# volivan239/raytracing-course-hw

Measured on AMD Instinct MI355X. Metric: Msamples/sec at 1920x1080x256spp, higher is better.
Workload: dtype f32; 1 GPU; synth_room_v1_1920x1080x256; scene=synth_room_v1 (seed 20241223), triangles=268816, emissive_triangles=4204, width=1920, height=1080, spp=256, ray_depth=6, parallelism=pixel tiles 32x32 round-robin over 1 GPU(s), bvh_nodes=265605, bvh_depth=24, light_bvh_depth=19, device_bytes=120573816

## Files before the change

raytracing-course-hw_amd/csrc/host/device_build.h:

```cpp
#pragma once
#include "../device/rt_types.h"
#include <cstdint>
#include <hip/hip_runtime.h>

namespace rtamd {

struct DeviceTree {
    GpuNode *nodes = nullptr;
    uint32_t *order = nullptr;
    uint8_t *last = nullptr;
    uint32_t n_nodes = 0, depth = 0;
    float build_ms = 0.f;
};

DeviceTree build_tree_on_device(const float *d_boxes, uint32_t n, float abs_pad, uint32_t max_depth);
void free_device_tree(DeviceTree &t);

void gather_records(const void *d_in, void *d_out, const DeviceTree &t, uint32_t n, uint32_t elem_bytes, int mark_word_offset, bool or_into_word = false);

void join_root_box(const GpuNode *d_nodes, float lo[3], float hi[3]);

GpuNode4Q *widen_nodes(const GpuNode *d_nodes, uint32_t n, const NodeGrid &grid, uint32_t &n_out, uint32_t &depth_out);

}
```

raytracing-course-hw_amd/csrc/rtamd_build.hip:

```cpp
#include "device/rt_bvh_build.h"
#include "device/rt_node_grid.h"
#include "host/device_build.h"
#include "host/fold_nodes.h"
#include "host/hip_check.h"
#include <cmath>
#include <stdexcept>
#include <string>
#include <vector>

namespace rtamd {

namespace {
__global__ void gather16_kernel(const float4 *in, float4 *out, const uint32_t *order, const uint8_t *last, uint32_t n, uint32_t quads, int mark_word, bool or_mark) {
    const uint32_t i = blockIdx.x * blockDim.x + threadIdx.x;
    if (i >= n) return;
    const float4 *src = in + (size_t)order[i] * quads;
    float4 *dst = out + (size_t)i * quads;
    for (uint32_t q = 0; q < quads; q++) dst[q] = src[q];
    if (mark_word >= 0) {
        uint32_t *w = reinterpret_cast<uint32_t *>(dst) + mark_word;
        const uint32_t mark = last[i] ? 1u : 0u;
        *w = or_mark ? ((*w & ~1u) | mark) : mark;
    }
}
}

void join_root_box(const GpuNode *d_nodes, float lo[3], float hi[3]) {
    GpuNode root;
    HIP_CHECK(hipMemcpy(&root, d_nodes, sizeof root, hipMemcpyDeviceToHost));
    auto join = [&](const float *l, const float *h) { for (int k = 0; k < 3; k++) { if (l[k] < lo[k]) lo[k] = l[k]; if (h[k] > hi[k]) hi[k] = h[k]; } };
    if ((uint32_t)root.child0 != 0xFFFFFFFFu) join(root.lo0, root.hi0);
    if ((uint32_t)root.child1 != 0xFFFFFFFFu) join(root.lo1, root.hi1);
}

GpuNode4Q *widen_nodes(const GpuNode *d_nodes, uint32_t n, const NodeGrid &grid, uint32_t &n_out, uint32_t &depth_out) {
    std::vector<GpuNode> nodes(n ? n : 1);
    if (n) HIP_CHECK(hipMemcpy(nodes.data(), d_nodes, (size_t)n * sizeof(GpuNode), hipMemcpyDeviceToHost));
    else { GpuNode e{}; e.child0 = e.child1 = (int32_t)0xFFFFFFFFu; nodes[0] = e; }
    std::vector<GpuNode4Q> wide;
    fold_nodes(nodes, grid, wide, depth_out);
    n_out = (uint32_t)wide.size();
    GpuNode4Q *out = nullptr;
    HIP_CHECK(hipMalloc((void **)&out, wide.size() * sizeof(GpuNode4Q)));
    if (hipMemcpy(out, wide.data(), wide.size() * sizeof(GpuNode4Q), hipMemcpyHostToDevice) != hipSuccess) { (void)hipFree(out); throw std::runtime_error("widen_nodes: upload failed"); }
    return out;
}

DeviceTree build_tree_on_device(const float *d_boxes, uint32_t n, float abs_pad, uint32_t max_depth) {
    DeviceTree t;
    if (n == 0) throw std::runtime_error("build_tree_on_device: no primitives");
    dev::BvbView B{};
    if (max_depth < 8 || max_depth > BVB_MAX_DEPTH) throw std::runtime_error("build_tree_on_device: max_depth out of range");
    B.boxes = d_boxes; B.n = n; B.abs_pad = abs_pad; B.max_depth = max_depth;
    const size_t max_open = (size_t)n / 2 + 2, max_nodes = 2 * (size_t)n + 2;
    std::vector<void *> temps;
    auto alloc = [&](size_t bytes, bool temp) { void *p = nullptr; HIP_CHECK(hipMalloc(&p, bytes)); if (temp) temps.push_back(p); return p; };
    try {
        B.prim_node = (uint32_t *)alloc((size_t)n * 4, true);
        B.nodes = (dev::BvbNode *)alloc(max_nodes * sizeof(dev::BvbNode), true);
        B.bins = (uint32_t *)alloc(max_open * BVB_NODE_BIN_WORDS * 4, true);
        B.dec = (dev::BvbDecision *)alloc(max_open * sizeof(dev::BvbDecision), true);
        B.open_cur = (uint32_t *)alloc(max_open * 4, true);
        B.open_next = (uint32_t *)alloc(max_open * 4, true);
        B.st = (dev::BvbState *)alloc(sizeof(dev::BvbState), true);
        t.order = B.order = (uint32_t *)alloc((size_t)n * 4, false);
        t.last = (uint8_t *)alloc((size_t)n, false);
        hipEvent_t e0, e1;
        HIP_CHECK(hipEventCreate(&e0)); HIP_CHECK(hipEventCreate(&e1));
        hipStream_t stream = 0;
        HIP_CHECK(hipEventRecord(e0, stream));
        HIP_CHECK(hipMemsetAsync(B.nodes, 0, 2 * sizeof(dev::BvbNode), stream));
        HIP_CHECK(hipMemsetAsync(B.bins, 0, max_open * BVB_NODE_BIN_WORDS * 4, stream));
        HIP_CHECK(hipMemsetAsync(t.last, 0, n, stream));
        const uint32_t prim_blocks = (n + 255) / 256, prim_wgs = (n + BVB_THREADS - 1) / BVB_THREADS, open_blocks = (uint32_t)((max_open + 255) / 256);
        hipLaunchKernelGGL(dev::bvb_init_kernel, dim3(prim_blocks), dim3(256), 0, stream, B);
        hipLaunchKernelGGL(dev::bvb_root_kernel, dim3(1), dim3(64), 0, stream, B);
        for (int level = 0; level <= (int)max_depth; level++) {
            hipLaunchKernelGGL(dev::bvb_bin_kernel, dim3(prim_wgs), dim3(BVB_THREADS), 0, stream, B);
            hipLaunchKernelGGL(dev::bvb_split_kernel, dim3(open_blocks), dim3(256), 0, stream, B);
            hipLaunchKernelGGL(dev::bvb_number_kernel, dim3(1), dim3(BVB_THREADS), 0, stream, B);
            hipLaunchKernelGGL(dev::bvb_assign_kernel, dim3(prim_wgs), dim3(BVB_THREADS), 0, stream, B);
            std::swap(B.open_cur, B.open_next);
            hipLaunchKernelGGL(dev::bvb_next_level_kernel, dim3(1), dim3(64), 0, stream, B);
            if ((level & 7) == 7) {
                dev::BvbState st;
                HIP_CHECK(hipMemcpyAsync(&st, B.st, sizeof st, hipMemcpyDeviceToHost, stream));
                HIP_CHECK(hipStreamSynchronize(stream));
                if (st.n_open == 0) break;
            }
        }
        hipLaunchKernelGGL(dev::bvb_layout_kernel, dim3(1), dim3(BVB_THREADS), 0, stream, B);
        dev::BvbState st;
        HIP_CHECK(hipMemcpyAsync(&st, B.st, sizeof st, hipMemcpyDeviceToHost, stream));
        HIP_CHECK(hipStreamSynchronize(stream));
        if (st.n_open != 0 || st.n_leaf_slots != n || st.n_nodes > max_nodes)
            throw std::runtime_error("build_tree_on_device: inconsistent tree (open " + std::to_string(st.n_open) + ", slots " + std::to_string(st.n_leaf_slots) + " of " + std::to_string(n) + ")");
        t.n_nodes = st.n_inner ? st.n_inner : 1u;
        t.depth = st.max_depth;
        t.nodes = B.out_nodes = (GpuNode *)alloc((size_t)t.n_nodes * sizeof(GpuNode), false);
        const uint32_t node_blocks = (st.n_nodes + 255) / 256;
        hipLaunchKernelGGL(dev::bvb_place_kernel, dim3(prim_blocks), dim3(256), 0, stream, B);
        hipLaunchKernelGGL(dev::bvb_emit_kernel, dim3(node_blocks), dim3(256), 0, stream, B);
        hipLaunchKernelGGL(dev::bvb_marks_kernel, dim3(node_blocks), dim3(256), 0, stream, B, t.last);
        HIP_CHECK(hipEventRecord(e1, stream));
        HIP_CHECK(hipStreamSynchronize(stream));
        HIP_CHECK(hipGetLastError());
        HIP_CHECK(hipEventElapsedTime(&t.build_ms, e0, e1));
        (void)hipEventDestroy(e0); (void)hipEventDestroy(e1);
    } catch (...) {
        for (void *p : temps) (void)hipFree(p);
        free_device_tree(t);
        throw;
    }
    for (void *p : temps) (void)hipFree(p);
    return t;
}

void free_device_tree(DeviceTree &t) {
    if (t.nodes) (void)hipFree(t.nodes);
    if (t.order) (void)hipFree(t.order);
    if (t.last) (void)hipFree(t.last);
    t.nodes = nullptr; t.order = nullptr; t.last = nullptr;
}

void gather_records(const void *d_in, void *d_out, const DeviceTree &t, uint32_t n, uint32_t elem_bytes, int mark_word_offset, bool or_into_word) {
    if (elem_bytes % 16) throw std::runtime_error("gather_records: record size must be a multiple of 16");
    hipLaunchKernelGGL(gather16_kernel, dim3((n + 255) / 256), dim3(256), 0, 0, (const float4 *)d_in, (float4 *)d_out, t.order, t.last, n, elem_bytes / 16, mark_word_offset, or_into_word);
    HIP_CHECK(hipGetLastError());
}

}
```

raytracing-course-hw_amd/csrc/rtamd_scene.hip:

```cpp
#include <hip/hip_runtime.h>
#include <cmath>
#include <cstdio>
#include <cstdlib>
#include <cstring>
#include <memory>
#include <string>
#include <vector>
#include "../../include/rtamd.h"
#include "host/host_scene.h"
#include "host/png.h"
#include "host/scene_prep.h"
#include "host/shared_prep.h"
#include "host/device_build.h"
#include "host/knobs.h"
#include "host/rt_scene.h"
#include "device/rt_node_grid.h"

namespace rtamd {
static thread_local std::string g_last_error;
void set_error(const std::string &msg) { g_last_error = msg; }
}
using namespace rtamd;

namespace {

struct OwnedTree {
    DeviceTree t;
    ~OwnedTree() { free_device_tree(t); }
};

template <class Rec>
DeviceTree build_leaf_ordered(rt_scene *s, const float *d_boxes, const Rec *d_records, uint32_t n, float box_pad, uint32_t depth_cap,
                              int mark_word, bool or_into_word, const Rec *&gathered) {
    OwnedTree tree;
    tree.t = build_tree_on_device(d_boxes, n, box_pad, depth_cap);
    OwnedDev out;
    HIP_CHECK(hipMalloc(&out.p, (size_t)n * sizeof(Rec)));
    gather_records(d_records, out.p, tree.t, n, sizeof(Rec), mark_word, or_into_word);
    HIP_CHECK(hipDeviceSynchronize());
    s->allocations.reserve(s->allocations.size() + 2);
    s->allocations.push_back(tree.t.nodes);
    s->allocations.push_back(out.p);
    gathered = (const Rec *)out.release();
    DeviceTree t = tree.t;
    t.order = nullptr; t.last = nullptr;
    tree.t.nodes = nullptr;
    return t;
}

void make_walk_nodes(rt_scene *s, const float cam_pos[3], const GpuNode *nodes, uint32_t n_nodes, const GpuNode *light_nodes, uint32_t n_light_nodes,
                     bool join_light_root, NodeGrid &grid, const GpuNode4Q *&nodes4, const GpuNode4Q *&light_nodes4, uint64_t &bytes) {
    float glo[3], ghi[3];
    for (int k = 0; k < 3; k++) glo[k] = ghi[k] = cam_pos[k];
    join_root_box(nodes, glo, ghi);
    if (join_light_root) join_root_box(light_nodes, glo, ghi);
    grid = make_node_grid(glo, ghi);
    uint32_t n4 = 0, n4l = 0, depth4 = 0;
    s->allocations.push_back(widen_nodes(nodes, n_nodes, grid, n4, depth4));
    nodes4 = (const GpuNode4Q *)s->allocations.back();
    s->allocations.push_back(widen_nodes(light_nodes, n_light_nodes, grid, n4l, depth4));
    light_nodes4 = (const GpuNode4Q *)s->allocations.back();
    bytes += ((uint64_t)n4 + n4l) * sizeof(GpuNode4Q);
}

template <class View> void set_camera(View &V, const rt_scene_desc &desc) {
    for (int k = 0; k < 3; k++) {
        V.cam_pos[k] = desc.camera.position[k]; V.cam_right[k] = desc.camera.right[k];
        V.cam_up[k] = desc.camera.up[k]; V.cam_fwd[k] = desc.camera.forward[k];
        V.bg[k] = desc.bg_color[k];
    }
}

int finish_scene(std::unique_ptr<rt_scene> &s, rt_scene **out, uint64_t bytes, double t0, double t1) {
    HIP_CHECK(hipMalloc((void **)&s->d_work_counter, 64));
    s->allocations.push_back(s->d_work_counter);
    HIP_CHECK(hipMalloc((void **)&s->d_counters, CNT_BYTES));
    s->allocations.push_back(s->d_counters);
    HIP_CHECK(hipEventCreate(&s->ev_start));
    HIP_CHECK(hipEventCreate(&s->ev_stop));
    HIP_CHECK(hipDeviceSynchronize());
    s->info.device_bytes = bytes;
    s->info.prep_ms = t1 - t0; s->info.upload_ms = now_ms() - t1;
    *out = s.release();
    return RT_OK;
}

struct Uploader {
    rt_scene *s;
    uint64_t bytes = 0;
    template <class T> const T *operator()(const std::vector<T> &v) { s->allocations.push_back((void *)upload(v, bytes)); return (const T *)s->allocations.back(); }
};
template <class View> void upload_ref_trees(View &V, const PreparedTrees &P, Uploader &up) { V.ref_nodes = up(P.ref_nodes); V.ref_light_nodes = up(P.ref_light_nodes); }
void report_trees(rt_scene *s, const rt_scene_desc *desc, const PreparedTrees &P, uint32_t n_lights, uint32_t n_nodes, uint32_t bvh_depth) {
    s->light_order = P.light_order;
    s->info.n_triangles = desc->n_triangles; s->info.n_lights = n_lights;
    s->info.n_bvh_nodes = n_nodes; s->info.n_light_bvh_nodes = (uint32_t)P.light_nodes.size();
    s->info.bvh_depth = bvh_depth; s->info.light_bvh_depth = P.light_bvh_depth;
}

template <class View> void set_triangle_view(View &V, const rt_scene_desc &desc, const PreparedTriangles &P, uint32_t components) {
    V.box_c2 = P.box_c2; V.box_c2x = 1.25f * P.box_c2;
    V.cull_k = (float)env_float("RTAMD_CULL_K", 0.0078125);
    V.n_tris = desc.n_triangles;
    V.n_lights = (uint32_t)P.light_order.size();
    V.n_components = components + (V.n_lights ? 1u : 0u);
    V.n_lights_f = (float)V.n_lights; V.n_components_f = (float)V.n_components;
    set_camera(V, desc);
    V.tan_fov_y = (float)std::tan((double)(desc.camera.fov_y / 2));
}

int create_txt(const rt_scene_desc *desc, std::unique_ptr<rt_scene> &s, rt_scene **out, double t0) {
    PreparedSceneTxt T;
    prepare_scene_txt(*desc, T);
    PreparedScene5 P5;
    prepare_scene_hw5(*desc, P5);
    Uploader up{s.get()};
    s->txt_has_triangles = T.has_triangles;
    SceneViewTxt &V = s->viewt;
    V.prims = up(T.prims);
    V.n_prims = desc->n_primitives;
    set_camera(V, *desc);
    V.tan_fov_x = (float)std::tan((double)(desc->camera.fov_x / 2));
    V.tan_fov_x_f = tanf(desc->camera.fov_x / 2);
    V.n_lights = desc->n_lights;
    if (desc->n_lights) V.lights = up(T.lights);
    for (int k = 0; k < 3; k++) V.ambient[k] = desc->ambient_light[k];
    V.n_light_prims = (uint32_t)T.light_prims.size();
    if (!T.light_prims.empty()) V.light_prims = up(T.light_prims);
    SceneView5 &V5 = s->view5;
    V5.nodes = up(P5.nodes);
    V5.figs = up(P5.figs);
    V5.light_nodes = up(P5.light_nodes);
    upload_ref_trees(V5, P5, up);
    if (!P5.lights.empty()) V5.lights = up(P5.lights);
    V5.n_figs = (uint32_t)P5.figs.size(); V5.n_nonplanes = P5.n_nonplanes; V5.n_lights = (uint32_t)P5.lights.size();
    set_camera(V5, *desc);
    V5.tan_fov_x = V.tan_fov_x;
    report_trees(s.get(), desc, P5, V5.n_lights, (uint32_t)P5.nodes.size(), P5.bvh_depth);
    s->flavor = RT_INTEGRATOR_HW3;
    return finish_scene(s, out, up.bytes, t0, t0);
}

int create_hw6(const rt_scene_desc *desc, std::unique_ptr<rt_scene> &s, rt_scene **out, double t0) {
    const bool tree_on_device = desc->n_triangles >= 64 && !env_flag("RTAMD_HOST_BVH");
    PreparedScene6 P6;
    prepare_scene_hw6(*desc, P6, tree_on_device);
    uint32_t bvh_depth = P6.bvh_depth, n_nodes = (uint32_t)P6.nodes.size();
    double t1 = now_ms();
    Uploader up{s.get()};
    SceneView6 &V = s->view6;
    if (tree_on_device) {
        uint64_t scratch = 0;
        OwnedDev d_load(upload(P6.tris, up.bytes));
        OwnedDev d_boxes(upload(P6.boxes8, scratch));
        const DeviceTree t = build_leaf_ordered(s.get(), (const float *)d_boxes.p, (const Tri6 *)d_load.p, desc->n_triangles, P6.box_pad, 28,
                                                13, false, V.tris);
        V.nodes = t.nodes;
        up.bytes += (uint64_t)t.n_nodes * sizeof(GpuNode);
        bvh_depth = t.depth;
        n_nodes = t.n_nodes;
        s->info.bvh_build_ms = t.build_ms; s->info.bvh_on_device = 1;
    } else {
        V.nodes = up(P6.nodes);
        V.tris = up(P6.tris);
    }
    if (bvh_depth > RT6_STACK_SIZE - 2 || P6.light_bvh_depth > RT6_STACK_SIZE - 2 || P6.fast_light_bvh_depth > RT6_STACK_SIZE - 2)
        return fail(RT_ERR_LIMIT, "scene BVH deeper than the kernel's traversal stack (" + std::to_string(bvh_depth) + "/" +
                                      std::to_string(P6.light_bvh_depth) + ")");
    s->hw6_lds_stack = bvh_depth <= RT6_LDS_STACK && P6.fast_light_bvh_depth <= RT6_LDS_STACK;
    s->hw6_pt_stack = bvh_depth <= P6_STACK && P6.fast_light_bvh_depth <= P6_STACK;
    V.light_nodes = up(P6.light_nodes);
    V.lights = up(P6.lights);
    V.fast_light_nodes = up(P6.fast_light_nodes);
    V.fast_lights = up(P6.fast_lights);
    V.light_ref = up(P6.light_ref);
    upload_ref_trees(V, P6, up);
    V.ref_tris = up(P6.ref_tris);
    V.tri_box = up(P6.tri_box);
    set_triangle_view(V, *desc, P6, 1u);
    V.exact_boxes = env_flag("RTAMD_NO_EXACT_BOXES") ? 0u : 1u;
    V.light_sep = up(P6.light_sep);
    V.materials = up(P6.materials);
    s->view.tan_fov_y = V.tan_fov_y;
    s->flavor = RT_INTEGRATOR_HW6;
    make_walk_nodes(s.get(), V.cam_pos, V.nodes, n_nodes, V.fast_light_nodes, (uint32_t)P6.fast_light_nodes.size(), true,
                    V.grid, V.nodes4, V.fast_light_nodes4, up.bytes);
    report_trees(s.get(), desc, P6, V.n_lights, n_nodes, bvh_depth);
    return finish_scene(s, out, up.bytes, t0, t1);
}

int create_hw8(const rt_scene_desc *desc, std::unique_ptr<rt_scene> &s, rt_scene **out, double t0, SharedPrep *shared) {
    if (desc->build_flags & ~RT_BUILD_DEVICE_BVH) return fail(RT_ERR_INVALID_ARG, "rt_scene_create: unknown build_flags");
    const bool fast_build = (desc->build_flags & RT_BUILD_DEVICE_BVH) && desc->n_triangles >= 64;
    const bool walk_tree_on_device = desc->n_triangles >= 64 && (fast_build || !env_flag("RTAMD_HOST_BVH"));
    PreparedScene P_local;
    if (shared) std::call_once(shared->once, [&] { try { prepare_scene(*desc, shared->P, fast_build); } catch (...) { shared->error = std::current_exception(); } });
    else prepare_scene(*desc, P_local, fast_build);
    if (shared && shared->error) std::rethrow_exception(shared->error);
    const PreparedScene &P = shared ? shared->P : P_local;
    uint32_t bvh_depth = P.bvh_depth, n_nodes = (uint32_t)P.nodes.size();
    double t1 = now_ms();
    Uploader up{s.get()};
    SceneView &V = s->view;
    V.tri_isect = up(P.isect);
    V.tri_shade = up(P.shade);
    V.tri_box = up(P.tri_box);
    if (walk_tree_on_device) {
        const uint32_t n = desc->n_triangles;
        uint64_t scratch = 0;
        OwnedDev d_walk_box;
        if (!P.walk_box.empty()) d_walk_box.p = upload(P.walk_box, scratch);
        const DeviceTree t = build_leaf_ordered(s.get(), d_walk_box.p ? (const float *)d_walk_box.p : V.tri_box, V.tri_isect, n, P.box_pad, P8_STACK,
                                                11, true, V.tri_walk);
        V.nodes = t.nodes;
        up.bytes += (uint64_t)t.n_nodes * sizeof(GpuNode) + (uint64_t)n * sizeof(TriIsect);
        bvh_depth = t.depth;
        n_nodes = t.n_nodes;
        s->info.bvh_build_ms = t.build_ms; s->info.bvh_on_device = 1;
    } else {
        V.nodes = up(P.nodes);
        V.tri_walk = V.tri_isect;
    }
    if (P.bvh_depth > RT_STACK_SIZE - 2)
        return fail(RT_ERR_LIMIT, "the reference's scene BVH is deeper than the exact walk's stack (" + std::to_string(P.bvh_depth) + ")");
    if (bvh_depth > RT_STACK_SIZE - 2 || P.light_bvh_depth > RT_STACK_SIZE - 2)
        return fail(RT_ERR_LIMIT, "scene BVH deeper than the kernel's traversal stack (" + std::to_string(bvh_depth) + "/" +
                                      std::to_string(P.light_bvh_depth) + ")");
    V.light_nodes = up(P.light_nodes);
    V.light_sep = up(P.light_sep);
    upload_ref_trees(V, P, up);
    set_triangle_view(V, *desc, P, 2u);
    V.box_c2x *= (float)env_float("RTAMD_C2X_SCALE", 1.0);
    V.exact_boxes = (env_flag("RTAMD_NO_EXACT_BOXES") || fast_build) ? 0u : 1u;
    if (env_flag("RTAMD_DIAG_LOOKBEHIND_ONLY")) V.exact_boxes = 2u;
    V.n_tripwire_groups = (V.exact_boxes != 1u || env_flag("RTAMD_NO_TRIPWIRES")) ? 0u : P.n_tripwire_groups;
    V.tripwires = V.n_tripwire_groups ? up(P.tripwires) : nullptr;
    V.lights = up(P.lights);
    uint32_t n_light_walk_nodes = 0;
    {
        const uint32_t nl = (uint32_t)P.lights.size();
        const LightRec *ordered = nullptr;
        std::vector<LightRec> tagged = P.lights;
        for (uint32_t i = 0; i < nl; i++) tagged[i].isect.pad = (i << 1) | (tagged[i].isect.pad ? 1u : 0u);
        if (nl >= 64 && !env_flag("RTAMD_HOST_LIGHT_BVH")) {
            uint64_t scratch = 0;
            OwnedDev d_tagged(upload(tagged, up.bytes));
            OwnedDev d_lbox(upload(P.light_walk_box, scratch));
            const DeviceTree lt = build_leaf_ordered(s.get(), (const float *)d_lbox.p, (const LightRec *)d_tagged.p, nl, P.box_pad, 16,
                                                     11, true, ordered);
            V.light_walk_nodes = lt.nodes;
            up.bytes += (uint64_t)lt.n_nodes * sizeof(GpuNode);
            s->light_walk_depth = lt.depth;
            n_light_walk_nodes = lt.n_nodes;
        } else {
            V.light_walk_nodes = V.light_nodes;
            n_light_walk_nodes = (uint32_t)P.light_nodes.size();
            ordered = up(tagged);
            s->light_walk_depth = P.light_bvh_depth;
        }
        OwnedDev whole(s->allocations.back());
        s->allocations.pop_back();
        const size_t n_rec = nl ? nl : 1u;
        char *pair = nullptr;
        HIP_CHECK(hipMalloc((void **)&pair, n_rec * sizeof(LightRec)));
        s->allocations.push_back(pair);
        char *rest = pair + n_rec * sizeof(TriIsect);
        HIP_CHECK(hipMemcpy2D(pair, sizeof(TriIsect), ordered, sizeof(LightRec), sizeof(TriIsect), n_rec, hipMemcpyDeviceToDevice));
        HIP_CHECK(hipMemcpy2D(rest, sizeof(LightRest), (const char *)ordered + sizeof(TriIsect), sizeof(LightRec), sizeof(LightRest), n_rec, hipMemcpyDeviceToDevice));
        V.lights_walk_test = (const TriIsect *)pair;
        V.lights_walk_rest = (const LightRest *)rest;
    }
    V.materials = up(P.materials);
    V.images = up(P.images);
    V.texels = up(P.texels);
    V.srgb_lut = up(std::vector<float>(P.srgb_lut, P.srgb_lut + 256));
    V.n_nodes = n_nodes;
    V.last_level_emission_only = 1;
    for (uint32_t i = 0; i < desc->n_materials; i++) {
        const rt_material &m = desc->materials[i];
        if (!(m.metallic_factor >= 0 && m.metallic_factor <= 1 && m.base_color[0] >= 0 && m.base_color[1] >= 0 && m.base_color[2] >= 0))
            V.last_level_emission_only = 0;
    }
    if (env_flag("RTAMD_NO_LAST_LEVEL_SHORTCUT")) V.last_level_emission_only = 0;
    V.env_image = P.env_image;
    if (!walk_arrays_fit(desc->n_triangles, V.n_lights, n_nodes, n_light_walk_nodes))
        return fail(RT_ERR_LIMIT, "the scene's triangles, lights or tree nodes do not fit the walkers' 32-bit offsets (2^24 records, 4 GiB per array)");
    make_walk_nodes(s.get(), V.cam_pos, V.nodes, n_nodes, V.light_walk_nodes, n_light_walk_nodes, n_light_walk_nodes != 0,
                    V.grid, V.nodes4, V.light_walk_nodes4, up.bytes);
    report_trees(s.get(), desc, P, V.n_lights, n_nodes, bvh_depth);
    return finish_scene(s, out, up.bytes, t0, t1);
}

}

int rtamd::scene_create_shared(const rt_scene_desc *desc, rt_scene **out, rtamd::SharedPrep *shared) {
    if (!desc || !out) return fail(RT_ERR_INVALID_ARG, "rt_scene_create: null argument");
    if (desc->struct_size != sizeof(rt_scene_desc)) return fail(RT_ERR_INVALID_ARG, "rt_scene_create: struct_size mismatch (ABI skew)");
    *out = nullptr;
    int ndev = 0;
    if (hipGetDeviceCount(&ndev) != hipSuccess || ndev == 0)
        return fail(RT_ERR_NO_DEVICE, "rt_scene_create: no HIP device available (this library has no CPU fallback)");
    return guarded("", [&]() -> int {
        std::unique_ptr<rt_scene> s(new rt_scene());
        HIP_CHECK(hipGetDevice(&s->device));
        hipDeviceProp_t prop;
        HIP_CHECK(hipGetDeviceProperties(&prop, s->device));
        s->n_cus = prop.multiProcessorCount > 0 ? prop.multiProcessorCount : 256;
        const double t0 = now_ms();
        if (desc->n_triangles == 0 && (desc->n_primitives > 0 || (desc->camera.fov_x != 0.f && desc->camera.fov_y == 0.f))) return create_txt(desc, s, out, t0);
        if (desc->n_triangles && !desc->normals) return create_hw6(desc, s, out, t0);
        return create_hw8(desc, s, out, t0, shared);
    });
}

extern "C" {

const char *rt_last_error(void) { return g_last_error.c_str(); }

int rt_scene_create(const rt_scene_desc *desc, rt_scene **out) { return rtamd::scene_create_shared(desc, out, nullptr); }

void rt_scene_destroy(rt_scene *scene) { delete scene; }

int rt_scene_get_info(const rt_scene *scene, rt_scene_info *info) {
    if (!scene || !info) return fail(RT_ERR_INVALID_ARG, "rt_scene_get_info: null argument");
    *info = scene->info;
    return RT_OK;
}

int rt_scene_get_light_order(const rt_scene *scene, uint32_t *out, uint32_t capacity) {
    if (!scene || (!out && capacity)) return fail(RT_ERR_INVALID_ARG, "rt_scene_get_light_order: null argument");
    if (capacity < scene->light_order.size()) return fail(RT_ERR_INVALID_ARG, "rt_scene_get_light_order: buffer too small");
    memcpy(out, scene->light_order.data(), scene->light_order.size() * sizeof(uint32_t));
    return (int)scene->light_order.size();
}

int rt_host_prepare_orders(const rt_scene_desc *desc, int integrator, uint32_t *figure_order, uint32_t figure_capacity,
                           uint32_t *light_order, uint32_t light_capacity) {
    if (!desc || desc->struct_size != sizeof(rt_scene_desc)) return fail(RT_ERR_INVALID_ARG, "rt_host_prepare_orders: bad desc");
    return guarded("rt_host_prepare_orders: ", [&]() -> int {
        auto answer = [&](const PreparedTrees &P) -> int {
            if ((figure_order && figure_capacity < P.figure_order.size()) || (light_order && light_capacity < P.light_order.size())) return fail(RT_ERR_INVALID_ARG, "rt_host_prepare_orders: buffer too small");
            if (figure_order) memcpy(figure_order, P.figure_order.data(), P.figure_order.size() * sizeof(uint32_t));
            if (light_order) memcpy(light_order, P.light_order.data(), P.light_order.size() * sizeof(uint32_t));
            return (int)P.light_order.size();
        };
        if (integrator == RT_INTEGRATOR_HW8 || integrator == RT_INTEGRATOR_HW7) { PreparedScene P; prepare_scene(*desc, P); return answer(P); }
        if (integrator == RT_INTEGRATOR_HW6) { PreparedScene6 P; prepare_scene_hw6(*desc, P); return answer(P); }
        if (integrator == RT_INTEGRATOR_HW5) { PreparedScene5 P; prepare_scene_hw5(*desc, P); return answer(P); }
        return fail(RT_ERR_UNSUPPORTED, "rt_host_prepare_orders: integrator must be HW5, HW6, HW7 or HW8");
    });
}

int rt_unshard(const rt_render_params *p, const void *shard_buf, size_t elem_size, void *full_image) {
    if (!p || !shard_buf || !full_image || (elem_size != 1 && elem_size != 4)) return fail(RT_ERR_INVALID_ARG, "rt_unshard: bad argument");
    return guarded("rt_unshard: ", [&]() -> int {
    RenderView R{};
    std::string err;
    if (!resolve_tiles(p, R, err)) return fail(RT_ERR_INVALID_ARG, "rt_unshard: " + err);
    const uint8_t *src = (const uint8_t *)shard_buf;
    uint8_t *dst = (uint8_t *)full_image;
    size_t px = 3 * elem_size;
    if (R.shard_count <= 1) { memcpy(dst, src, (size_t)R.width * R.height * px); return RT_OK; }
    for (uint32_t st = 0; st < R.n_shard_tiles; st++) {
        int tx0, ty0, w, h;
        shard_tile_rect(R, st, tx0, ty0, w, h);
        for (int ly = 0; ly < h; ly++)
            memcpy(dst + ((size_t)(ty0 + ly) * R.width + tx0) * px, src + (((size_t)st * R.tile_h + ly) * R.tile_w) * px, (size_t)w * px);
    }
    return RT_OK;
    });
}

int rt_load_gltf(const char *path, int flavor, rt_host_scene **out) {
    if (!path || !out) return fail(RT_ERR_INVALID_ARG, "rt_load_gltf: null argument");
    *out = nullptr;
    return guarded(std::string("rt_load_gltf(") + path + "): ", [&]() -> int { *out = load_gltf(path, flavor); return RT_OK; }, RT_ERR_PARSE);
}
int rt_load_txt(const char *path, int flavor, rt_host_scene **out, int32_t *w, int32_t *h, int32_t *samples, int32_t *depth) {
    if (!path || !out) return fail(RT_ERR_INVALID_ARG, "rt_load_txt: null argument");
    *out = nullptr;
    return guarded(std::string("rt_load_txt(") + path + "): ", [&]() -> int { *out = load_txt(path, flavor, w, h, samples, depth); return RT_OK; }, RT_ERR_PARSE);
}
int rt_host_scene_set_environment(rt_host_scene *hs, const char *image_path) {
    if (!hs || !image_path) return fail(RT_ERR_INVALID_ARG, "rt_host_scene_set_environment: null argument");
    return guarded("", [&]() -> int {
        int w, h;
        load_image_rgb8(image_path, w, h, hs->env_data);
        hs->env = rt_image{w, h, nullptr};
        hs->has_env = true;
        hs->finalize();
        return RT_OK;
    }, RT_ERR_IO);
}
const rt_scene_desc *rt_host_scene_desc(const rt_host_scene *hs) { return hs ? &hs->desc : nullptr; }
void rt_host_scene_free(rt_host_scene *hs) { delete hs; }

int rt_write_ppm(const char *path, int32_t width, int32_t height, const uint8_t *rgb8) {
    if (!path || !rgb8 || width <= 0 || height <= 0) return fail(RT_ERR_INVALID_ARG, "rt_write_ppm: bad argument");
    FILE *f = fopen(path, "wb");
    if (!f) return fail(RT_ERR_IO, std::string("rt_write_ppm: cannot open ") + path);
    fprintf(f, "P6\n%d %d\n255\n", width, height);
    size_t n = (size_t)width * height * 3;
    bool ok = fwrite(rgb8, 1, n, f) == n;
    ok = (fclose(f) == 0) && ok;
    return ok ? RT_OK : fail(RT_ERR_IO, std::string("rt_write_ppm: short write to ") + path);
}
int rt_decode_png(const char *path, int32_t *width, int32_t *height, uint8_t **rgb) {
    if (!path || !width || !height || !rgb) return fail(RT_ERR_INVALID_ARG, "rt_decode_png: null argument");
    return guarded("", [&]() -> int {
        std::vector<uint8_t> px;
        int w, h;
        load_image_rgb8(path, w, h, px);
        *rgb = (uint8_t *)malloc(px.size());
        if (!*rgb) return fail(RT_ERR_IO, "rt_decode_png: out of memory");
        memcpy(*rgb, px.data(), px.size());
        *width = w; *height = h;
        return RT_OK;
    }, RT_ERR_IO);
}
void rt_free(void *p) { free(p); }

}
```

Measured before the change: 544.9 Msamples/s.

## Collapse binary BVH into 4-wide nodes with SAH-optimal dynamic-programming cuts

Replaces the fixed level-pair fold of the binary BVH into 4-wide quantized nodes with a dynamic program. For each subtree it picks which binary nodes to open so that each wide node's children minimize the expected number of traversal steps, weighted by surface area. The goal is fewer visited wide nodes per ray in both the scene and light trees. It falls back to the level-pair fold if the result is larger, costlier or deeper, and pads the array to the pair-fold size. Host build time grows and the traversal order of children changes.

Result: no change. 549.3 Msamples/s, median of 2 (+0.8%).

```diff
diff --git a/raytracing-course-hw_amd/csrc/host/collapse_nodes.h b/raytracing-course-hw_amd/csrc/host/collapse_nodes.h
--- /dev/null
+++ b/raytracing-course-hw_amd/csrc/host/collapse_nodes.h
@@ -0,0 +1,173 @@
+#pragma once
+#include <cstdint>
+#include <limits>
+#include <stdexcept>
+#include <string>
+#include <vector>
+#include "fold_nodes.h"
+
+namespace rtamd {
+
+struct CollapsedNodes {
+    std::vector<GpuNode4Q> wide;
+    uint32_t depth = 0;
+    uint32_t pair_nodes = 0;
+    double pair_cost = 0.0;
+    double cost = 0.0;
+    uint32_t pair_cuts = 0;
+    bool fell_back = false;
+};
+
+inline CollapsedNodes collapse_nodes(const std::vector<GpuNode> &nodes, const NodeGrid &grid) {
+    constexpr uint32_t EMPTY = 0xFFFFFFFFu, LEAF = 0x80000000u;
+    constexpr double INF = std::numeric_limits<double>::infinity();
+    CollapsedNodes out;
+    std::vector<GpuNode4Q> pair;
+    uint32_t pair_depth = 0;
+    fold_nodes(nodes, grid, pair, pair_depth);
+    out.pair_nodes = (uint32_t)pair.size();
+
+    struct Edge { const float *lo, *hi; uint32_t child; };
+    auto edge = [&](uint32_t x, int side) { const GpuNode &b = nodes[x]; return side ? Edge{b.lo1, b.hi1, (uint32_t)b.child1} : Edge{b.lo0, b.hi0, (uint32_t)b.child0}; };
+    auto inner = [&](uint32_t child) { return !(child & LEAF); };
+    auto half_area = [](const double lo[3], const double hi[3]) {
+        const double d[3] = {hi[0] - lo[0], hi[1] - lo[1], hi[2] - lo[2]};
+        return d[0] * d[1] + d[1] * d[2] + d[2] * d[0];
+    };
+
+    double root_area = 0.0;
+    {
+        double lo[3] = {INF, INF, INF}, hi[3] = {-INF, -INF, -INF};
+        for (int side = 0; side < 2; side++) {
+            const Edge e = edge(0, side);
+            if (e.child == EMPTY) continue;
+            for (int a = 0; a < 3; a++) { if (e.lo[a] < lo[a]) lo[a] = e.lo[a]; if (e.hi[a] > hi[a]) hi[a] = e.hi[a]; }
+        }
+        if (lo[0] <= hi[0]) root_area = half_area(lo, hi);
+        if (!(root_area > 0.0)) root_area = 1.0;
+    }
+
+    struct Best { double area = 1.0, W = 0.0, G[5]; uint32_t height = 1, below[5], levels = 1; };
+    std::vector<Best> best(nodes.size());
+    std::vector<uint32_t> order{0u};
+    std::vector<uint8_t> reached(nodes.size(), 0);
+    reached[0] = 1;
+    for (size_t i = 0; i < order.size(); i++)
+        for (int side = 0; side < 2; side++) {
+            const Edge e = edge(order[i], side);
+            if (!inner(e.child)) continue;
+            if (reached[e.child]) throw std::runtime_error("collapse_nodes: the two-box nodes do not form a tree");
+            reached[e.child] = 1; order.push_back(e.child);
+            const double lo[3] = {e.lo[0], e.lo[1], e.lo[2]}, hi[3] = {e.hi[0], e.hi[1], e.hi[2]};
+            best[e.child].area = half_area(lo, hi) / root_area;
+        }
+    struct Forest { double F[5]; };
+    auto forest_of = [&](uint32_t child) {
+        Forest f;
+        if (child == EMPTY) { for (int k = 0; k < 5; k++) f.F[k] = 0.0; }
+        else if (!inner(child)) { f.F[0] = INF; for (int k = 1; k < 5; k++) f.F[k] = 0.0; }
+        else { const Best &c = best[child]; f.F[0] = c.G[0]; for (int k = 1; k < 5; k++) f.F[k] = c.W < c.G[k] ? c.W : c.G[k]; }
+        return f;
+    };
+    auto pick_split = [&](const Forest &f0, const Forest &f1, int k) {
+        int j_best = 0; double v_best = INF;
+        for (int j = 0; j <= k; j++) { const double v = f0.F[j] + f1.F[k - j]; if (v < v_best) { v_best = v; j_best = j; } }
+        return j_best;
+    };
+    auto fewest = [](const Best &b, int k) { while (k > 0 && b.G[k - 1] <= b.G[k]) k--; return k; };
+    auto pick_open = [&](const Best &c, int k, int &k_open) { k_open = fewest(c, k); return c.G[k] < c.W || (c.G[k] == c.W && k_open <= 1); };
+    auto levels_under = [&](uint32_t child, int k) -> uint32_t {
+        if (!inner(child)) return 0;
+        const Best &c = best[child];
+        int k_open;
+        return pick_open(c, k, k_open) ? c.below[k_open] : c.levels;
+    };
+    for (size_t i = order.size(); i-- > 0;) {
+        const uint32_t x = order[i];
+        Best &b = best[x];
+        const uint32_t c0 = edge(x, 0).child, c1 = edge(x, 1).child;
+        const Forest f0 = forest_of(c0), f1 = forest_of(c1);
+        for (uint32_t c : {c0, c1}) if (inner(c) && best[c].height + 1 > b.height) b.height = best[c].height + 1;
+        for (int k = 0; k < 5; k++) {
+            const int j = pick_split(f0, f1, k);
+            b.G[k] = f0.F[j] + f1.F[k - j];
+            const uint32_t l0 = levels_under(c0, j), l1 = levels_under(c1, k - j);
+            b.below[k] = l0 > l1 ? l0 : l1;
+        }
+        b.W = b.area + b.G[4];
+        b.levels = 1 + b.below[fewest(b, 4)];
+    }
+
+    {
+        std::vector<uint32_t> todo{0u};
+        for (size_t i = 0; i < todo.size(); i++) {
+            out.pair_cost += best[todo[i]].area;
+            for (int side = 0; side < 2; side++) {
+                const uint32_t c = edge(todo[i], side).child;
+                if (!inner(c)) continue;
+                for (int s2 = 0; s2 < 2; s2++) { const uint32_t g = edge(c, s2).child; if (inner(g)) todo.push_back(g); }
+            }
+        }
+    }
+
+    auto levels_of = [&](uint32_t x) { const uint32_t pairs = (best[x].height + 1) / 2; return best[x].levels < pairs ? best[x].levels : pairs; };
+    std::vector<uint32_t> source{0u}, level{1u};
+    struct Todo { Edge e; int k; };
+    std::vector<Todo> todo;
+    uint32_t misfits = 0;
+    out.depth = 1;
+    out.wide.reserve(pair.size());
+    for (size_t w = 0; w < source.size(); w++) {
+        const uint32_t x = source[w];
+        const uint32_t levels_below = pair_depth - level[w];
+        Edge e[4]; int ne = 0;
+        auto split = [&](uint32_t at, int k) {
+            const int j = pick_split(forest_of(edge(at, 0).child), forest_of(edge(at, 1).child), k);
+            todo.push_back(Todo{edge(at, 1), k - j});
+            todo.push_back(Todo{edge(at, 0), j});
+        };
+        todo.clear();
+        split(x, fewest(best[x], 4));
+        while (!todo.empty()) {
+            const Todo t = todo.back(); todo.pop_back();
+            if (t.e.child == EMPTY) continue;
+            int k_open;
+            if (inner(t.e.child) && pick_open(best[t.e.child], t.k, k_open)) split(t.e.child, k_open);
+            else e[ne++] = t.e;
+        }
+        bool fits = true;
+        for (int k = 0; k < ne; k++) if (inner(e[k].child) && levels_of(e[k].child) > levels_below) fits = false;
+        if (!fits) {
+            ne = 0; out.pair_cuts++;
+            for (int side = 0; side < 2; side++) {
+                const Edge c = edge(x, side);
+                if (c.child == EMPTY) continue;
+                if (!inner(c.child)) { e[ne++] = c; continue; }
+                for (int s2 = 0; s2 < 2; s2++) { const Edge g = edge(c.child, s2); if (g.child != EMPTY) e[ne++] = g; }
+            }
+        }
+        out.cost += best[x].area;
+        GpuNode4Q q;
+        for (int k = 0; k < 4; k++) {
+            if (k >= ne) { q.rec[k][0] = q.rec[k][1] = q.rec[k][2] = 0u; q.rec[k][3] = EMPTY; continue; }
+            bool on_grid = true;
+            for (int a = 0; a < 3; a++) q.rec[k][a] = grid_axis_word(e[k].lo[a], e[k].hi[a], grid.lo[a], grid.step[a], on_grid);
+            if (!on_grid) misfits++;
+            uint32_t child = e[k].child;
+            if (inner(child)) {
+                source.push_back(child); level.push_back(level[w] + 1);
+                if (level[w] + 1 > out.depth) out.depth = level[w] + 1;
+                child = (uint32_t)(source.size() - 1);
+            }
+            q.rec[k][3] = child;
+        }
+        out.wide.push_back(q);
+    }
+    if (misfits) throw std::runtime_error("collapse_nodes: " + std::to_string(misfits) + " node boxes do not fit the scene's grid");
+    if (out.wide.size() > pair.size() || out.cost > out.pair_cost || out.depth > pair_depth) {
+        out.wide.swap(pair); out.depth = pair_depth; out.cost = out.pair_cost; out.fell_back = true;
+    }
+    return out;
+}
+
+}
diff --git a/raytracing-course-hw_amd/csrc/host/device_build.h b/raytracing-course-hw_amd/csrc/host/device_build.h
--- a/raytracing-course-hw_amd/csrc/host/device_build.h
+++ b/raytracing-course-hw_amd/csrc/host/device_build.h
@@ -20,6 +20,6 @@
 
 void join_root_box(const GpuNode *d_nodes, float lo[3], float hi[3]);
 
-GpuNode4Q *widen_nodes(const GpuNode *d_nodes, uint32_t n, const NodeGrid &grid, uint32_t &n_out, uint32_t &depth_out);
+GpuNode4Q *widen_nodes(const GpuNode *d_nodes, uint32_t n, const NodeGrid &grid, const char *what, uint32_t &n_out, uint32_t &depth_out);
 
 }
diff --git a/raytracing-course-hw_amd/csrc/rtamd_build.hip b/raytracing-course-hw_amd/csrc/rtamd_build.hip
--- a/raytracing-course-hw_amd/csrc/rtamd_build.hip
+++ b/raytracing-course-hw_amd/csrc/rtamd_build.hip
@@ -1,9 +1,12 @@
 #include "device/rt_bvh_build.h"
 #include "device/rt_node_grid.h"
 #include "host/device_build.h"
-#include "host/fold_nodes.h"
+#include "host/collapse_nodes.h"
 #include "host/hip_check.h"
+#include "host/knobs.h"
+#include <chrono>
 #include <cmath>
+#include <cstdio>
 #include <stdexcept>
 #include <string>
 #include <vector>
@@ -33,13 +36,25 @@
     if ((uint32_t)root.child1 != 0xFFFFFFFFu) join(root.lo1, root.hi1);
 }
 
-GpuNode4Q *widen_nodes(const GpuNode *d_nodes, uint32_t n, const NodeGrid &grid, uint32_t &n_out, uint32_t &depth_out) {
+GpuNode4Q *widen_nodes(const GpuNode *d_nodes, uint32_t n, const NodeGrid &grid, const char *what, uint32_t &n_out, uint32_t &depth_out) {
     std::vector<GpuNode> nodes(n ? n : 1);
     if (n) HIP_CHECK(hipMemcpy(nodes.data(), d_nodes, (size_t)n * sizeof(GpuNode), hipMemcpyDeviceToHost));
     else { GpuNode e{}; e.child0 = e.child1 = (int32_t)0xFFFFFFFFu; nodes[0] = e; }
-    std::vector<GpuNode4Q> wide;
-    fold_nodes(nodes, grid, wide, depth_out);
-    n_out = (uint32_t)wide.size();
+    const auto t0 = std::chrono::steady_clock::now();
+    CollapsedNodes c = collapse_nodes(nodes, grid);
+    const double ms = std::chrono::duration<double, std::milli>(std::chrono::steady_clock::now() - t0).count();
+    std::vector<GpuNode4Q> &wide = c.wide;
+    if (env_flag("RTAMD_DEBUG_COUNTERS")) {
+        size_t used = 0;
+        for (const GpuNode4Q &q : wide) for (int k = 0; k < 4; k++) used += q.rec[k][3] != 0xFFFFFFFFu;
+        fprintf(stderr, "[rtamd] %s walk tree: %zu wide nodes (level pairs %u), %.2f records used per node, %u levels, expected steps %.4f (level pairs %.4f), %u level-pair cuts for depth%s, %.2f ms\n",
+                what, wide.size(), c.pair_nodes, (double)used / (double)wide.size(), c.depth, c.cost, c.pair_cost, c.pair_cuts, c.fell_back ? ", the level-pair fold kept" : "", ms);
+    }
+    depth_out = c.depth;
+    n_out = c.pair_nodes;
+    GpuNode4Q unused;
+    for (int k = 0; k < 4; k++) { unused.rec[k][0] = unused.rec[k][1] = unused.rec[k][2] = 0u; unused.rec[k][3] = 0xFFFFFFFFu; }
+    wide.resize(c.pair_nodes, unused);
     GpuNode4Q *out = nullptr;
     HIP_CHECK(hipMalloc((void **)&out, wide.size() * sizeof(GpuNode4Q)));
     if (hipMemcpy(out, wide.data(), wide.size() * sizeof(GpuNode4Q), hipMemcpyHostToDevice) != hipSuccess) { (void)hipFree(out); throw std::runtime_error("widen_nodes: upload failed"); }
diff --git a/raytracing-course-hw_amd/csrc/rtamd_scene.hip b/raytracing-course-hw_amd/csrc/rtamd_scene.hip
--- a/raytracing-course-hw_amd/csrc/rtamd_scene.hip
+++ b/raytracing-course-hw_amd/csrc/rtamd_scene.hip
@@ -56,9 +56,9 @@
     if (join_light_root) join_root_box(light_nodes, glo, ghi);
     grid = make_node_grid(glo, ghi);
     uint32_t n4 = 0, n4l = 0, depth4 = 0;
-    s->allocations.push_back(widen_nodes(nodes, n_nodes, grid, n4, depth4));
+    s->allocations.push_back(widen_nodes(nodes, n_nodes, grid, "scene", n4, depth4));
     nodes4 = (const GpuNode4Q *)s->allocations.back();
-    s->allocations.push_back(widen_nodes(light_nodes, n_light_nodes, grid, n4l, depth4));
+    s->allocations.push_back(widen_nodes(light_nodes, n_light_nodes, grid, "light", n4l, depth4));
     light_nodes4 = (const GpuNode4Q *)s->allocations.back();
     bytes += ((uint64_t)n4 + n4l) * sizeof(GpuNode4Q);
 }
```
